# BBischof/ESRecsys

Hardware: AMD Instinct MI355X
Metric: training pairs/sec (higher is better)
Workload: dtype f32; 1 GPU; inbatch: V=1000000 x D=128 fp32 tables, B=8192, sparse Adagrad; score_precision=auto -> f16x2, ids=uniform, parallelism=single

## Files before the change

esrecsys_amd/csrc/esr_inbatch2h.hip:

```cpp
#include "esr_inbatch_mfma.h"
#include "esr_segment.h"
#include <atomic>
#include <type_traits>
#include <time.h>

namespace esr {

typedef _Float16 f16x8 __attribute__((ext_vector_type(8)));
typedef _Float16 f16x2 __attribute__((ext_vector_type(2)));

constexpr int kHLseOff = 2 * kPlaneBytes;
constexpr int kHBufBytes = kHLseOff + 4 * 256;
constexpr float kHOptHead = 4.0f;
constexpr float kHOverflow = 60000.0f;
constexpr int kHBufs = 3;
constexpr float kHPexp = 14.0f;
constexpr float kHBoundSafe = 14.0f;
constexpr int kHScaleWords = 8;

#define H_MFMA(a, b, c) __builtin_amdgcn_mfma_f32_32x32x16_f16((a), (b), (c), 0, 0, 0)
#define H_SB() __builtin_amdgcn_sched_barrier(0)
#define H_DMA_BARRIER()                                 \
  {                                                     \
    asm volatile("s_waitcnt vmcnt(0)" ::: "memory");    \
// ... 100 lines not shown
  const s16x8 both = {lo[0], lo[1], lo[2], lo[3], hi[0], hi[1], hi[2], hi[3]};
  ta[G][DB][PL] = __builtin_bit_cast(f16x8, both);
}
template <int G, class TA>
__device__ __forceinline__ void trh_frag_n(int f, TA& ta, const uint32_t (&tc)[4][2]) {
  switch (f) {
    case 0: trh_frag<G, 0>(ta, tc); break;
    case 1: trh_frag<G, 1>(ta, tc); break;
    case 2: trh_frag<G, 2>(ta, tc); break;
    case 3: trh_frag<G, 3>(ta, tc); break;
    case 4: trh_frag<G, 4>(ta, tc); break;
    case 5: trh_frag<G, 5>(ta, tc); break;
    case 6: trh_frag<G, 6>(ta, tc); break;
    default: trh_frag<G, 7>(ta, tc); break;
  }
}

template <int K>
__device__ __forceinline__ uint32_t dmah_off0(int64_t B, int64_t chunk, int t) {
  const int within = (t + 256 * K) & 511;
  const int row = within >> 4, seg = (within & 15) ^ swz16(row);
  return (uint32_t)((((int64_t)(K >> 1) * B + chunk * 32 + row) * k3D + seg * 8) * 2);
}
template <int K>
__device__ __forceinline__ void dmah_piece(const char* __restrict__ base, uint32_t off, char* buf, int w) {
  __builtin_amdgcn_global_load_lds((gptr_t)(base + off), (lptr_t)(buf + K * 4096 + w * 1024), 16, 0, 0);
}
#define H_DP(K, G, BUF) dmah_piece<K>(baseY, G, (BUF), w)
#define H_DMA_ADVANCE()                                                                    \
  {                                                                                        \
    const uint32_t step_ = (dpos + 1 == nc) ? (uint32_t)(8192 - nc * 8192) : 8192u;        \
    dpos = (dpos + 1 == nc) ? 0 : dpos + 1;                                                \
    g0 += step_; g1 += step_; g2 += step_; g3 += step_;                                    \
  }
#define H_DMA_CHUNK(BUF) { H_DP(0, g0, BUF); H_DP(1, g1, BUF); H_DP(2, g2, BUF); H_DP(3, g3, BUF); H_DMA_ADVANCE(); }

__global__ __launch_bounds__(256) void prep2h_kernel(RowSrc X0, RowSrc X1, float* __restrict__ amax,
                                                    float* __restrict__ diag) {
  __shared__ float red[8];
  const int t = threadIdx.x;
  const int64_t grow = (int64_t)blockIdx.x * 32 + (t >> 3);
  const int d0 = (t & 7) * 16;
  float mq = 0.f, mc = 0.f, dot = 0.f;
#pragma unroll
  for (int q = 0; q < 4; ++q) {
    const float4 f = rowsrc_load4(X0, grow, d0 + 4 * q);
    const float4 g = rowsrc_load4(X1, grow, d0 + 4 * q);
    mq = fmaxf(mq, fmaxf(fmaxf(fabsf(f.x), fabsf(f.y)), fmaxf(fabsf(f.z), fabsf(f.w))));
    mc = fmaxf(mc, fmaxf(fmaxf(fabsf(g.x), fabsf(g.y)), fmaxf(fabsf(g.z), fabsf(g.w))));
    dot = fmaf(f.x, g.x, fmaf(f.y, g.y, fmaf(f.z, g.z, fmaf(f.w, g.w, dot))));
  }
  dot += __shfl_xor(dot, 1, 64);
  dot += __shfl_xor(dot, 2, 64);
  dot += __shfl_xor(dot, 4, 64);
  if ((t & 7) == 0) diag[grow] = dot;
#pragma unroll
  for (int o = 32; o > 0; o >>= 1) {
    mq = fmaxf(mq, __shfl_xor(mq, o, 64));
    mc = fmaxf(mc, __shfl_xor(mc, o, 64));
  }
  if ((t & 63) == 0) { red[t >> 6] = mq; red[4 + (t >> 6)] = mc; }
  __syncthreads();
  if (t == 0) {
    amax[blockIdx.x] = fmaxf(fmaxf(red[0], red[1]), fmaxf(red[2], red[3]));
    amax[gridDim.x + blockIdx.x] = fmaxf(fmaxf(red[4], red[5]), fmaxf(red[6], red[7]));
  }
}

__device__ __forceinline__ int scale_exp(float amax) {
  if (!(amax > 0.f) || !(amax < INFINITY)) return 0;
  int x;
  frexpf(amax, &x);
  const int e = 14 - x;
  return e < -100 ? -100 : (e > 100 ? 100 : e);
}

__global__ __launch_bounds__(256) void split2h_kernel(RowSrc X0, RowSrc X1, int64_t B, _Float16* __restrict__ R0,
                                                     _Float16* __restrict__ R1, const float* __restrict__ amax,
                                                     float* __restrict__ nrm, float* __restrict__ sc,
                                                     unsigned long long* __restrict__ loss_acc,
                                                     int* __restrict__ flags, int nflags) {
  __shared__ float red[8];
  if (blockIdx.x == 0 && blockIdx.y == 1)
    for (int i = threadIdx.x; i < nflags; i += 256) flags[i] = 0;
  if (blockIdx.x == 0 && blockIdx.y == 0 && threadIdx.x <= kLossWords) {
    loss_acc[threadIdx.x * 16] = 0ull;
    if (threadIdx.x == 0) loss_acc[8] = 0ull;
  }
  const int t = threadIdx.x, nchunks = gridDim.x;
  float mq = 0.f, mc = 0.f;
  for (int i = t; i < nchunks; i += 256) {
    mq = fmaxf(mq, amax[i]);
    mc = fmaxf(mc, amax[nchunks + i]);
  }
#pragma unroll
  for (int o = 32; o > 0; o >>= 1) {
    mq = fmaxf(mq, __shfl_xor(mq, o, 64));
    mc = fmaxf(mc, __shfl_xor(mc, o, 64));
  }
  if ((t & 63) == 0) { red[t >> 6] = mq; red[4 + (t >> 6)] = mc; }
  __syncthreads();
  mq = fmaxf(fmaxf(red[0], red[1]), fmaxf(red[2], red[3]));
  mc = fmaxf(fmaxf(red[4], red[5]), fmaxf(red[6], red[7]));
  const int eq = scale_exp(mq), ec = scale_exp(mc);
  if (blockIdx.x == 0 && blockIdx.y == 0 && t == 0) {
    sc[0] = ldexpf(1.f, -(eq + ec));
    sc[1] = ldexpf(1.f, -ec);
    sc[2] = ldexpf(1.f, -(eq + (int)kHPexp));
    sc[3] = ldexpf(1.f, eq);
    sc[4] = ldexpf(1.f, ec);
  }
  const RowSrc X = blockIdx.y ? X1 : X0;
  _Float16* R = blockIdx.y ? R1 : R0;
  const float mul = ldexpf(1.f, blockIdx.y ? ec : eq);
  const int chunk = blockIdx.x;
  const int row = t >> 3, d0 = (t & 7) * 16;
  const int64_t grow = (int64_t)chunk * 32 + row;
  float v[16];
#pragma unroll
  for (int q = 0; q < 4; ++q) {
    const float4 f = rowsrc_load4(X, grow, d0 + 4 * q);
    v[4 * q] = f.x; v[4 * q + 1] = f.y; v[4 * q + 2] = f.z; v[4 * q + 3] = f.w;
  }
  {
    float ss = 0.f;
#pragma unroll
    for (int e = 0; e < 16; ++e) ss = fmaf(v[e], v[e], ss);
    ss += __shfl_xor(ss, 1, 64);
    ss += __shfl_xor(ss, 2, 64);
    ss += __shfl_xor(ss, 4, 64);
    ss = fmaxf(ss, __shfl_xor(ss, 8, 64));
    ss = fmaxf(ss, __shfl_xor(ss, 16, 64));
    ss = fmaxf(ss, __shfl_xor(ss, 32, 64));
    if ((t & 63) == 0) nrm[((int64_t)blockIdx.y * gridDim.x + chunk) * 4 + (t >> 6)] = ss;
  }
  f16x8 p[2][2];
#pragma unroll
  for (int e = 0; e < 16; ++e) {
    const float xs = v[e] * mul;
    const _Float16 a = (_Float16)xs;
    const _Float16 b = (_Float16)(xs - (float)a);
    p[0][e >> 3][e & 7] = a;
    p[1][e >> 3][e & 7] = b;
  }
#pragma unroll
  for (int pl = 0; pl < 2; ++pl) {
    f16x8* dst = reinterpret_cast<f16x8*>(R + ((int64_t)pl * B + grow) * k3D + d0);
    dst[0] = p[pl][0];
    dst[1] = p[pl][1];
  }
}

constexpr unsigned long long kPollTicks = 300000000ull;
__device__ __forceinline__ unsigned amax_code(float amax) {
  if (!(amax > 0.f)) return 0u;
  if (!(amax < INFINITY)) return 255u;
  int x;
  frexpf(amax, &x);
  return (unsigned)min(max(x + 127, 1), 254);
}
__device__ __forceinline__ int scale_exp_code(unsigned code) {
  if (code == 0u || code == 255u) return 0;
  const int e = 14 - ((int)code - 127);
  return e < -100 ? -100 : (e > 100 ? 100 : e);
}

__global__ __launch_bounds__(256) void prepsplit2h_kernel(RowSrc X0, RowSrc X1, int64_t B, _Float16* __restrict__ R0,
                                                         _Float16* __restrict__ R1,
                                                         unsigned long long* __restrict__ ent,
                                                         unsigned long long token, float* __restrict__ diag,
                                                         float* __restrict__ nrm, float* __restrict__ sc,
                                                         unsigned long long* __restrict__ loss_acc,
                                                         int* __restrict__ flags, int nflags,
                                                         float* __restrict__ copy0, float* __restrict__ copy1,
                                                         unsigned* __restrict__ czero, int two_level) {
  __shared__ float red[8];
  __shared__ unsigned cred[8];
  const int t = threadIdx.x, chunk = blockIdx.x, nchunks = gridDim.x;
  if (chunk == 0 && t <= kLossWords) {
    loss_acc[t * 16] = 0ull;
    if (t == 0) loss_acc[8] = 0ull;
  }
  if (chunk == 1 || nchunks == 1)
    for (int i = t; i < nflags; i += 256) flags[i] = 0;
  if (czero && chunk == 0 && t < 16) czero[t] = 0u;
  const int row = t >> 3, d0 = (t & 7) * 16;
  const int64_t grow = (int64_t)chunk * 32 + row;
  float vq[16], vc[16];
  {
    const int64_t rq = X0.idx ? (int64_t)X0.idx[grow] : grow;
    const int64_t rc = X1.idx ? (int64_t)X1.idx[grow] : grow;
    RowSrc Y0 = X0, Y1 = X1;
    Y0.idx = nullptr; Y1.idx = nullptr;
#pragma unroll
    for (int q = 0; q < 4; ++q) {
      const float4 f = rowsrc_load4(Y0, rq, d0 + 4 * q);
      const float4 g = rowsrc_load4(Y1, rc, d0 + 4 * q);
      vq[4 * q] = f.x; vq[4 * q + 1] = f.y; vq[4 * q + 2] = f.z; vq[4 * q + 3] = f.w;
      vc[4 * q] = g.x; vc[4 * q + 1] = g.y; vc[4 * q + 2] = g.z; vc[4 * q + 3] = g.w;
      if (copy0 && d0 + 4 * q < X0.ld) *reinterpret_cast<float4*>(copy0 + grow * X0.ld + d0 + 4 * q) = f;
      if (copy1 && d0 + 4 * q < X1.ld) *reinterpret_cast<float4*>(copy1 + grow * X1.ld + d0 + 4 * q) = g;
    }
  }
  float mq = 0.f, mc = 0.f, dot = 0.f, ssq = 0.f, ssc = 0.f;
#pragma unroll
  for (int e = 0; e < 16; ++e) {
    mq = fmaxf(mq, fabsf(vq[e]));
    mc = fmaxf(mc, fabsf(vc[e]));
    dot = fmaf(vq[e], vc[e], dot);
    ssq = fmaf(vq[e], vq[e], ssq);
    ssc = fmaf(vc[e], vc[e], ssc);
  }
  dot += __shfl_xor(dot, 1, 64); dot += __shfl_xor(dot, 2, 64); dot += __shfl_xor(dot, 4, 64);
  ssq += __shfl_xor(ssq, 1, 64); ssq += __shfl_xor(ssq, 2, 64); ssq += __shfl_xor(ssq, 4, 64);
  ssc += __shfl_xor(ssc, 1, 64); ssc += __shfl_xor(ssc, 2, 64); ssc += __shfl_xor(ssc, 4, 64);
  if ((t & 7) == 0) diag[grow] = dot;
#pragma unroll
  for (int o = 8; o < 64; o <<= 1) {
    ssq = fmaxf(ssq, __shfl_xor(ssq, o, 64));
    ssc = fmaxf(ssc, __shfl_xor(ssc, o, 64));
  }
  if ((t & 63) == 0) {
    nrm[((int64_t)0 * nchunks + chunk) * 4 + (t >> 6)] = ssq;
    nrm[((int64_t)1 * nchunks + chunk) * 4 + (t >> 6)] = ssc;
  }
#pragma unroll
  for (int o = 32; o > 0; o >>= 1) {
    mq = fmaxf(mq, __shfl_xor(mq, o, 64));
    mc = fmaxf(mc, __shfl_xor(mc, o, 64));
  }
  if ((t & 63) == 0) { red[t >> 6] = mq; red[4 + (t >> 6)] = mc; }
  __syncthreads();
  if (t == 0) {
    mq = fmaxf(fmaxf(red[0], red[1]), fmaxf(red[2], red[3]));
    mc = fmaxf(fmaxf(red[4], red[5]), fmaxf(red[6], red[7]));
    __hip_atomic_store(&ent[chunk], (token << 16) | (unsigned long long)(amax_code(mq) << 8 | amax_code(mc)),
                       __ATOMIC_RELAXED, __HIP_MEMORY_SCOPE_AGENT);
  }
  unsigned cq = 0u, cc = 0u;
  bool timed_out = false;
  const unsigned long long t_start = __builtin_amdgcn_s_memrealtime();
  const bool gatherer = chunk == 0 || !two_level;
  for (int i = gatherer ? t : (t == 0 ? nchunks : nchunks + 1); i < (gatherer ? nchunks : nchunks + 1); i += 256) {
    unsigned long long v;
    while (((v = __hip_atomic_load(&ent[i], __ATOMIC_RELAXED, __HIP_MEMORY_SCOPE_AGENT)) >> 16) != token) {
      if (__builtin_amdgcn_s_memrealtime() - t_start > kPollTicks) { timed_out = true; break; }
      __builtin_amdgcn_s_sleep(4);
    }
    cq = max(cq, (unsigned)(v >> 8) & 255u);
    cc = max(cc, (unsigned)v & 255u);
  }
  if (timed_out) atomicOr(reinterpret_cast<unsigned*>(loss_acc + 8), 1u);
#pragma unroll
  for (int o = 32; o > 0; o >>= 1) {
    cq = max(cq, (unsigned)__shfl_xor((int)cq, o, 64));
    cc = max(cc, (unsigned)__shfl_xor((int)cc, o, 64));
  }
  if ((t & 63) == 0) { cred[t >> 6] = cq; cred[4 + (t >> 6)] = cc; }
  __syncthreads();
  cq = max(max(cred[0], cred[1]), max(cred[2], cred[3]));
  cc = max(max(cred[4], cred[5]), max(cred[6], cred[7]));
  if (two_level && chunk == 0 && t == 0)
    __hip_atomic_store(&ent[nchunks], (token << 16) | (unsigned long long)(cq << 8 | cc), __ATOMIC_RELAXED,
                       __HIP_MEMORY_SCOPE_AGENT);
  const int eq = scale_exp_code(cq), ec = scale_exp_code(cc);
  if (chunk == 0 && t == 0) {
    sc[0] = ldexpf(1.f, -(eq + ec));
    sc[1] = ldexpf(1.f, -ec);
    sc[2] = ldexpf(1.f, -(eq + (int)kHPexp));
    sc[3] = ldexpf(1.f, eq);
    sc[4] = ldexpf(1.f, ec);
  }
#pragma unroll
  for (int m = 0; m < 2; ++m) {
    const float mul = ldexpf(1.f, m ? ec : eq);
    _Float16* R = m ? R1 : R0;
    f16x8 p[2][2];
#pragma unroll
    for (int e = 0; e < 16; ++e) {
      const float xs = (m ? vc[e] : vq[e]) * mul;
      const _Float16 a = (_Float16)xs;
      const _Float16 b = (_Float16)(xs - (float)a);
      p[0][e >> 3][e & 7] = a;
      p[1][e >> 3][e & 7] = b;
    }
#pragma unroll
    for (int pl = 0; pl < 2; ++pl) {
      f16x8* dst = reinterpret_cast<f16x8*>(R + ((int64_t)pl * B + grow) * k3D + d0);
      dst[0] = p[pl][0];
      dst[1] = p[pl][1];
    }
  }
}

constexpr int kHRmGroup = 4, kHRmRing = 4, kHRmOwned = 256;
template <bool FULL>
__device__ __forceinline__ float rowmax2h_sweep(const char* __restrict__ baseY, char* lds, int64_t B, int64_t c0, int nc,
                                                const f16x8 (&bx0)[2][8], const f16x8 (&bx1)[2][8], int t, int w, int j,
                                                int h) {
  constexpr int kG = FULL ? kHRmGroup / 2 : kHRmGroup;
  constexpr int kSlotChunk = (FULL ? 2 : 1) * kPlaneBytes, kSlot = kG * kSlotChunk;
  constexpr int kDmaPerGroup = kG * (FULL ? 4 : 2);
  const uint32_t g0 = dmah_off0<0>(B, c0, t), g1 = dmah_off0<1>(B, c0, t);
  const uint32_t g2 = dmah_off0<2>(B, c0, t), g3 = dmah_off0<3>(B, c0, t);
  const int ngroups = (nc + kG - 1) / kG;
#define H_RM_FETCH(GI)                                                                       \
  _Pragma("unroll") for (int k = 0; k < kG; ++k) {                                          \
    const int ch_ = min((GI) * kG + k, nc - 1);                                             \
    char* dst_ = lds + ((GI) % kHRmRing) * kSlot + k * kSlotChunk;                          \
    const uint32_t adv_ = (uint32_t)ch_ * 8192u;                                            \
    H_DP(0, g0 + adv_, dst_); H_DP(1, g1 + adv_, dst_);                                     \
    if (FULL) { H_DP(2, g2 + adv_, dst_); H_DP(3, g3 + adv_, dst_); }                       \
  }
#pragma unroll
  for (int gi = 0; gi < kHRmRing - 1; ++gi) { H_RM_FETCH(gi); }
  float ma = -INFINITY, mb = -INFINITY;
  for (int gi = 0; gi < ngroups; ++gi) {
    asm volatile("s_waitcnt vmcnt(%0)" ::"n"((kHRmRing - 2) * kDmaPerGroup) : "memory");
    __syncthreads();
    H_RM_FETCH(gi + kHRmRing - 1);
#pragma unroll
    for (int k = 0; k < kG; ++k) {
      if (gi * kG + k < nc) {
        const char* buf = lds + (gi % kHRmRing) * kSlot + k * kSlotChunk;
        f32x16 sa = {0.f, 0.f, 0.f, 0.f, 0.f, 0.f, 0.f, 0.f, 0.f, 0.f, 0.f, 0.f, 0.f, 0.f, 0.f, 0.f};
        f32x16 sb = sa;
#pragma unroll
        for (int s = 0; s < 8; ++s) {
          const int off = j * 256 + (((2 * s + h) ^ swz16(j)) << 4);
          const f16x8 a1 = *reinterpret_cast<const f16x8*>(buf + off);
          if (FULL) {
            const f16x8 a2 = *reinterpret_cast<const f16x8*>(buf + off + kPlaneBytes);
            sa = H_MFMA(a2, bx0[0][s], sa);
            sb = H_MFMA(a2, bx0[1][s], sb);
            sa = H_MFMA(a1, bx1[0][s], sa);
            sb = H_MFMA(a1, bx1[1][s], sb);
          }
          sa = H_MFMA(a1, bx0[0][s], sa);
          sb = H_MFMA(a1, bx0[1][s], sb);
        }
#pragma unroll
        for (int r = 0; r < 16; ++r) { ma = fmaxf(ma, sa[r]); mb = fmaxf(mb, sb[r]); }
      }
    }
  }
#undef H_RM_FETCH
  asm volatile("s_waitcnt vmcnt(0)" ::: "memory");
  const float mine = h == 0 ? ma : mb, other = h == 0 ? mb : ma;
  return fmaxf(mine, __shfl_xor(other, 32, 64));
}

__global__ __launch_bounds__(256) void rowmax2h_kernel(const _Float16* __restrict__ Xr, const _Float16* __restrict__ Yr,
                                                      int64_t B, int nsplit, float sl2, const float* __restrict__ nrm,
                                                      const float* __restrict__ sc, float* __restrict__ part_mr) {
  __shared__ __attribute__((aligned(16))) char lds[kHRmRing * kHRmGroup * kPlaneBytes];
  const int t = threadIdx.x, lane = t & 63;
  const int w = __builtin_amdgcn_readfirstlane(t >> 6);
  const int j = lane & 31, h = lane >> 5;
  const int ob = blockIdx.x / nsplit, split = blockIdx.x % nsplit;
  const int64_t wrow = (int64_t)ob * kHRmOwned + w * 64;
  const int64_t xrow = wrow + 32 * h + j;
  const bool live = wrow < B;
  float bound;
  {
    const int nslots = (int)(B / k3Chunk) * 4;
    float mq = 0.f, mc = 0.f;
    for (int i = t; i < nslots; i += 256) {
      mq = fmaxf(mq, nrm[i]);
      mc = fmaxf(mc, nrm[nslots + i]);
    }
#pragma unroll
    for (int o = 32; o > 0; o >>= 1) {
      mq = fmaxf(mq, __shfl_xor(mq, o, 64));
      mc = fmaxf(mc, __shfl_xor(mc, o, 64));
    }
    float* red = reinterpret_cast<float*>(lds);
    if (lane == 0) { red[w] = mq; red[4 + w] = mc; }
    __syncthreads();
    mq = fmaxf(fmaxf(red[0], red[1]), fmaxf(red[2], red[3]));
    mc = fmaxf(fmaxf(red[4], red[5]), fmaxf(red[6], red[7]));
    __syncthreads();
    bound = sqrtf(mq * mc) * fabsf(sl2);
    if (bound <= kHBoundSafe) {
      if (live) part_mr[(int64_t)split * B + xrow] = bound - kHPexp;
      return;
    }
  }
  const bool full = !(bound <= 1024.f);
  const float sl2s = sl2 * sc[0];
  const int nc = (int)(B / k3Chunk) / nsplit;
  const int64_t c0 = (int64_t)split * nc;
  const char* const baseY = reinterpret_cast<const char*>(Yr);
  f16x8 bx0[2][8], bx1[2][8];
#pragma unroll
  for (int u = 0; u < 2; ++u)
#pragma unroll
    for (int s = 0; s < 8; ++s) {
      const int64_t r = live ? wrow + 32 * u + j : 0;
      bx0[u][s] = *reinterpret_cast<const f16x8*>(Xr + r * k3D + 16 * s + 8 * h);
      bx1[u][s] = *reinterpret_cast<const f16x8*>(Xr + ((int64_t)B + r) * k3D + 16 * s + 8 * h);
      if (sl2 < 0.f) { bx0[u][s] = -bx0[u][s]; bx1[u][s] = -bx1[u][s]; }
    }
  const float m = full ? rowmax2h_sweep<true>(baseY, lds, B, c0, nc, bx0, bx1, t, w, j, h)
                       : rowmax2h_sweep<false>(baseY, lds, B, c0, nc, bx0, bx1, t, w, j, h);
  if (live) part_mr[(int64_t)split * B + xrow] = m * fabsf(sl2s) - kHPexp;
}

#ifndef H_S_ASM_LOADS
#define H_S_ASM_LOADS 1
#endif
template <int OFF>
__device__ __forceinline__ f16x8 lds_b128(uint32_t addr) {
  f16x8 v;
  asm volatile("ds_read_b128 %0, %1 offset:%2" : "=v"(v) : "v"(addr), "n"(OFF));
  return v;
}
#if H_S_ASM_LOADS
#define H_S_LD(P, OFFB) lds_b128<(P) * kPlaneBytes>(ap32_ + (uint32_t)(OFFB))
#define H_S_WAIT(N) { asm volatile("s_waitcnt lgkmcnt(%0)" ::"n"(N) : "memory"); }
#else
#define H_S_LD(P, OFFB) (*reinterpret_cast<const f16x8*>(ap0_ + (OFFB) + (P) * kPlaneBytes))
#define H_S_WAIT(N)
#endif
#define H_S_PHASE(NBUF, SA, VALU_ON)                                                                      \
  {                                                                                                       \
    _Pragma("unroll") for (int r_ = 0; r_ < 16; ++r_) SA[r_] = 0.f;                                       \
    const char* ap0_ = (NBUF) + j * 256;                                                                  \
    const uint32_t ap32_ = lds32 + (uint32_t)((NBUF) - lds) + (uint32_t)(j * 256);                        \
    (void)ap0_; (void)ap32_;                                                                              \
    const int sw_ = swz16(j);                                                                             \
    f16x8 a1_ = H_S_LD(0, (h ^ sw_) << 4);                                                                \
    f16x8 a2_ = H_S_LD(1, (h ^ sw_) << 4);                                                                \
    _Pragma("unroll") for (int s_ = 0; s_ < 8; ++s_) {                                                    \
      f16x8 n1_ = a1_, n2_ = a2_;                                                                         \
      if (s_ < 7) {                                                                                       \
        const int off_ = (((2 * (s_ + 1) + h) ^ sw_) << 4);                                               \
        n1_ = H_S_LD(0, off_);                                                                            \
        n2_ = H_S_LD(1, off_);                                                                            \
      }                                                                                                   \
      float e0_ = 0.f, e1_ = 0.f;                                                                         \
      f16x2 pa_ = {0, 0};                                                                                 \
      H_SB();                                                                                             \
      H_S_WAIT((s_ < 7 ? 2 : 0) + (((VALU_ON) && s_ >= 1) ? 2 : 0));                                      \
      H_SB();                                                                                             \
      SA = H_MFMA(a2_, bx[0][s_], SA);                                                                    \
// ... 924 lines not shown
    }
#undef CT_ROW_DMA
#undef CT_BAR
#undef CT_BAR_TOP_B
#undef CT_BAR_TOP
#undef CT_COMPUTE
#undef CT_LOAD
#undef CT_G1
#undef CT_G0
#undef CT_APPLY_FAC
#undef CT_LOAD_REFS
#undef CT_DMA_P
#undef CT_DMA_P_PIECE
#undef CT_DMA_Y
#undef CT_DMA_Y_PIECE
  };
  if (general) {
    sweep(std::true_type{});
  } else {
    sweep(std::false_type{});
    const float ce = cexp;
#pragma unroll
    for (int db = 0; db < 4; ++db)
#pragma unroll
      for (int r = 0; r < 16; ++r) acc[db][r] *= ce;
  }
  asm volatile("s_waitcnt vmcnt(0)" ::: "memory");
  __syncthreads();
  if (live) store_tile_via_lds<true>(lds + w * kTileLdsBytes, acc, part_O + ((int64_t)split * B + wrow) * k3D, lane);
}

__global__ __launch_bounds__(256) void fac2h_kernel(int64_t B, int nsplit, const float* __restrict__ part_m,
                                                   const float* __restrict__ part_l, float invl_scale,
                                                   float* __restrict__ fac, float* __restrict__ lse2 = nullptr,
                                                   float* __restrict__ lse_nat = nullptr) {
  const int64_t row = (int64_t)blockIdx.x * 256 + threadIdx.x;
  if (row >= B) return;
  float pm[8], pl[8];
#pragma unroll
  for (int s = 0; s < 8; ++s) {
    pm[s] = -INFINITY; pl[s] = 0.f;
    if (s < nsplit) {
      pm[s] = part_m[(int64_t)s * B + row];
      pl[s] = part_l[(int64_t)s * B + row];
    }
  }
  float M = pm[0], L = 0.f;
  float wt[8];
#pragma unroll
  for (int s = 1; s < 8; ++s) M = fmaxf(M, pm[s]);
#pragma unroll
  for (int s = 0; s < 8; ++s) {
    wt[s] = pm[s] == M ? 1.f : __builtin_amdgcn_exp2f(pm[s] - M);
    L = __fmaf_rn(pl[s], wt[s], L);
  }
  const float invL1 = __fdiv_rn(1.0f, L);
#pragma unroll
  for (int s = 0; s < 8; ++s)
    if (s < nsplit) fac[(int64_t)s * B + row] = __fmul_rn(__fmul_rn(invL1, invl_scale), wt[s]);
  if (lse2) {
    const float l2v = __fadd_rn(M, __builtin_amdgcn_logf(L));
    lse2[row] = l2v;
    if (lse_nat) lse_nat[row] = l2v * k3Ln2;
  }
}

constexpr int kCtExpShift = 11;
__global__ __launch_bounds__(256) void facscale2h_kernel(RowSrc X, int64_t B, int nsplit,
                                                        const float* __restrict__ part_m,
                                                        const float* __restrict__ part_l, float invl_scale,
                                                        const float* __restrict__ sc, float* __restrict__ fac,
                                                        float* __restrict__ lse2, float* __restrict__ lse_nat,
                                                        _Float16* __restrict__ Yt, int* __restrict__ cflags) {
  const int t = threadIdx.x, chunk = blockIdx.x;
  const int row = t >> 3, sl = t & 7, d0 = sl * 16;
  const int64_t grow = (int64_t)chunk * 32 + row;
  float v[16];
  {
    const int64_t r = X.idx ? (int64_t)X.idx[grow] : grow;
    RowSrc Y0 = X;
    Y0.idx = nullptr;
#pragma unroll
    for (int q = 0; q < 4; ++q) {
      const float4 f = rowsrc_load4(Y0, r, d0 + 4 * q);
      v[4 * q] = f.x; v[4 * q + 1] = f.y; v[4 * q + 2] = f.z; v[4 * q + 3] = f.w;
    }
  }
  const float pm_l = sl < nsplit ? part_m[(int64_t)sl * B + grow] : -INFINITY;
  const float pl_l = sl < nsplit ? part_l[(int64_t)sl * B + grow] : 0.f;
  float pm[8], pl[8];
  const int lane0 = (t & 63) & ~7;
#pragma unroll
  for (int s = 0; s < 8; ++s) {
    pm[s] = __shfl(pm_l, lane0 + s, 64);
    pl[s] = __shfl(pl_l, lane0 + s, 64);
  }
  float M = pm[0], L = 0.f;
  float wt[8];
#pragma unroll
  for (int s = 1; s < 8; ++s) M = fmaxf(M, pm[s]);
#pragma unroll
  for (int s = 0; s < 8; ++s) {
    wt[s] = pm[s] == M ? 1.f : __builtin_amdgcn_exp2f(pm[s] - M);
    L = __fmaf_rn(pl[s], wt[s], L);
  }
  const float invL1 = __fdiv_rn(1.0f, L);
  const float f1 = __fmul_rn(invL1, invl_scale);
  float wmine = 1.f;
#pragma unroll
  for (int s = 0; s < 8; ++s) wmine = s == sl ? wt[s] : wmine;
  const float fs = __fmul_rn(f1, wmine);
  if (sl < nsplit) {
    fac[(int64_t)sl * B + grow] = fs;
    if (fs != f1) cflags[sl] = 1;
  }
  if (sl == 0 && lse2) {
    const float l2v = __fadd_rn(M, __builtin_amdgcn_logf(L));
    lse2[grow] = l2v;
    if (lse_nat) lse_nat[grow] = l2v * k3Ln2;
  }
  const float mul = sc[3] * ldexpf(1.f, -kCtExpShift);
  float m = 0.f;
  f16x8 p[2][2];
#pragma unroll
  for (int e = 0; e < 16; ++e) {
    const float xs = __fmul_rn(v[e], f1) * mul;
    m = fmaxf(m, fabsf(xs));
    const _Float16 a = (_Float16)xs;
    const _Float16 b = (_Float16)(xs - (float)a);
    p[0][e >> 3][e & 7] = a;
    p[1][e >> 3][e & 7] = b;
  }
  m = fmaxf(m, __shfl_xor(m, 1, 64));
  m = fmaxf(m, __shfl_xor(m, 2, 64));
  m = fmaxf(m, __shfl_xor(m, 4, 64));
  if (sl < nsplit && (!(m < 60000.f) || (f1 != 0.f && m < kCtLive))) cflags[sl] = 1;
#pragma unroll
  for (int pl2 = 0; pl2 < 2; ++pl2) {
    f16x8* dst = reinterpret_cast<f16x8*>(Yt + ((int64_t)pl2 * B + grow) * k3D + d0);
    dst[0] = p[pl2][0];
    dst[1] = p[pl2][1];
  }
}

struct InbatchHWs {
  _Float16 *Qh, *Ch;
  float *part_O, *part_O2, *fac_side, *Qcopy, *Ccopy, *part_m, *part_mr, *part_l, *lse2, *fac, *Pmat, *nrm, *amax, *sc, *diag;
  int* flags;
  unsigned long long* loss_acc;
  unsigned long long* ent;
  _Float16* Qt;
  unsigned* czero;
  int* cflags;
};
constexpr int64_t kHMaxB = 16384;

static size_t inbatch2h_ws_layout(int64_t B, char* base, InbatchHWs* ws) {
  size_t off = 0;
  auto take = [&](size_t bytes) {
    char* p = base ? base + off : nullptr;
    off += align_up(bytes, 256);
    return p;
  };
  const size_t planes = (size_t)2 * B * k3D * 2;
  InbatchHWs w;
  w.Qh = (_Float16*)take(planes);
  w.Ch = (_Float16*)take(planes);
  w.part_O = (float*)take((size_t)8 * B * k3D * 4);
  w.part_O2 = (float*)take((size_t)8 * B * k3D * 4);
  w.fac_side = (float*)take((size_t)8 * B * 4);
  w.Qcopy = (float*)take((size_t)B * k3D * 4);
  w.Ccopy = (float*)take((size_t)B * k3D * 4);
  w.part_m = (float*)take((size_t)8 * B * 4);
  w.part_mr = (float*)take((size_t)8 * B * 4);
  w.part_l = (float*)take((size_t)8 * B * 4);
  w.lse2 = (float*)take((size_t)B * 4);
  w.fac = (float*)take((size_t)8 * B * 4);
  w.diag = (float*)take((size_t)B * 4);
  w.flags = (int*)take((size_t)8 * (B / k3Owned) * sizeof(int));
  w.Pmat = (float*)take((size_t)B * B * 4);
  w.loss_acc = (unsigned long long*)take(sizeof(unsigned long long) * 16 * (1 + kLossWords));
  w.nrm = (float*)take((size_t)2 * (B / k3Chunk) * 4 * sizeof(float));
  w.amax = (float*)take((size_t)2 * (B / k3Chunk) * sizeof(float));
  w.sc = (float*)take(kHScaleWords * sizeof(float));
  w.ent = (unsigned long long*)take((size_t)(B / k3Chunk + 1) * sizeof(unsigned long long));
  w.Qt = (_Float16*)take(planes);
  w.czero = (unsigned*)take(16 * sizeof(unsigned));
  w.cflags = reinterpret_cast<int*>(w.czero ? w.czero + 8 : nullptr);
  if (ws) *ws = w;
  return off;
}

static int inbatch2h_nsplit(int64_t B, int per_cu) {
  const int64_t owned_blocks = B / k3Owned, nchunks = B / k3Chunk;
  int best = 1;
  for (int s = 1; s <= 8; ++s)
    if (nchunks % s == 0 && owned_blocks * s <= 320 * per_cu) best = s;
  return best;
}

struct InbatchUpdate {
  void* tables[2];
  float* accums[2];
  int64_t row_offsets[3];
  int dtype;
  const int32_t* sorted_vids;
  const int32_t* perm;
  float* grad_rows;
  float lr, eps;
  bool skip_long;
};

static bool inbatch_events(hipEvent_t* fork, hipEvent_t* join) {
  constexpr int kMaxDev = 16;
  static thread_local hipEvent_t ev[kMaxDev][2] = {};
  int dev = 0;
  if (hipGetDevice(&dev) != hipSuccess || dev < 0 || dev >= kMaxDev) return false;
  for (int i = 0; i < 2; ++i)
    if (!ev[dev][i] && hipEventCreateWithFlags(&ev[dev][i], hipEventDisableTiming) != hipSuccess) return false;
  *fork = ev[dev][0];
  *join = ev[dev][1];
  return true;
}

}

using namespace esr;

extern "C" {

#ifdef H_TIMING
int esr_ib2h_debug_read(unsigned long long* host) {
  return (int)hipMemcpyFromSymbol(host, HIP_SYMBOL(esr_ib2h_dbg), sizeof(unsigned long long) * 8192);
}
#endif

size_t esr_inbatch2h_workspace_bytes(int64_t B, int D) {
  (void)D;
  if (B <= 0 || B > kHMaxB) return 256;
  return inbatch2h_ws_layout(B, nullptr, nullptr);
}

static int inbatch2h_run(const char* who, RowSrc Qs, RowSrc Cs, const int32_t* gq_rows, const int32_t* gc_rows, int64_t B,
                         int D, float scale, float regularization, float batch_size, float* loss, float* lse,
                         float* gQ, float* gC, void* workspace, size_t workspace_bytes, esr_stream_t stream,
                         hipStream_t side = nullptr, const InbatchUpdate* upd = nullptr) {
  if (!(B > 0 && B % k3Owned == 0 && B <= kHMaxB)) {
    set_error("%s: B=%lld must be a positive multiple of 128, at most %lld (larger batches: the bf16x3 entry point)",
              who, (long long)B, (long long)kHMaxB);
    return ESR_EINVAL;
  }
  if (!(D > 0 && D <= k3D && D % 4 == 0)) {
    set_error("%s: D=%d not supported (a multiple of 4, at most 128; wider rows: the f32 entry point)", who, D);
    return ESR_EINVAL;
  }
  if (!(Qs.base && Cs.base && loss && gQ && gC)) {
    set_error("%s: null pointer", who);
    return ESR_EINVAL;
  }
  if (batch_size == 0.f) {
    set_error("%s: batch_size must be non-zero", who);
    return ESR_EINVAL;
  }
  if ((((uintptr_t)Qs.base | (uintptr_t)Cs.base | (uintptr_t)gQ | (uintptr_t)gC) & 15) != 0) {
    set_error("%s: matrices must be 16-byte aligned", who);
    return ESR_EINVAL;
  }
  if (!workspace || workspace_bytes < esr_inbatch2h_workspace_bytes(B, D) || ((uintptr_t)workspace & 15)) {
    set_error("%s: workspace %zu bytes < %zu required (or misaligned)", who, workspace_bytes,
              esr_inbatch2h_workspace_bytes(B, D));
    return ESR_EWORKSPACE;
  }
  hipStream_t st = as_stream(stream);
  InbatchHWs ws;
  inbatch2h_ws_layout(B, (char*)workspace, &ws);
  const float inv_bs = 1.0f / batch_size, sl2 = scale * k3Log2e;
  const int nchunks = (int)(B / k3Chunk);
  const char* qcs = getenv("ESR_IB2H_Q_PER_CU");
  const int nsplit_q = inbatch2h_nsplit(B, qcs ? std::max(1, atoi(qcs)) : 2);
  const int pc_blocks = (int)cdiv(B, kCtOwned);
  int nsplit_c = 1;
  for (int sp = 1; sp <= 8; ++sp)
    if (nchunks % sp == 0 && pc_blocks * sp <= 320) nsplit_c = sp;
  const int grid_c = pc_blocks * nsplit_c;
  const int grid_q = (int)(B / k3Owned) * nsplit_q;
  const int mgrid = (int)std::min<int64_t>(k3MergeBlocks, cdiv(B, kBlock / 32));
  const char* refe = getenv("ESR_IB2H_REF");
  const int mode = (refe && refe[0] == 'r' && refe[1] == 'o') ? 0 : ((refe && refe[0] == 'r' && refe[1] == 'e') ? 2 : 1);
  const char* fe = getenv("ESR_IB2H_FUSED");
  const bool fused = !(fe && fe[0] == '0') && mode != 0;
  int nsplit_r = 1;
  hipEvent_t ev_fork = nullptr, ev_join = nullptr;
  const char* b16e = getenv("ESR_IB2H_BF16");
  const bool one_plane = fused && ((Qs.bf16 && Cs.bf16 && !(b16e && b16e[0] == 't')) || (b16e && b16e[0] == 'f'));
  const bool overlapped = fused && !one_plane && side != nullptr && side != st && inbatch_events(&ev_fork, &ev_join);
  const char* mue = getenv("ESR_IB2H_MERGE_UPDATE");
  const bool merge_upd = fused && !overlapped && upd != nullptr && upd->skip_long && D == k3D && Qs.ld == k3D &&
                         Cs.ld == k3D && !(mue && mue[0] == '0');
  auto merging_update = [&](int nsplit_of_c, const float* part_O_of_c) -> int {
    InbatchMergeArgs a;
    a.part_O[0] = ws.part_O; a.part_O[1] = part_O_of_c;
    a.nsplit[0] = nsplit_q; a.nsplit[1] = nsplit_of_c;
    a.oscale[0] = ws.sc + 1; a.oscale[1] = ws.sc + 2;
    a.partner[0] = ws.Ccopy; a.partner[1] = ws.Qcopy;
    a.part_m = ws.part_m; a.part_l = ws.part_l;
    a.B = B;
    a.scale = scale; a.lam = regularization; a.inv_bs = inv_bs;
    a.loss_acc = ws.loss_acc; a.loss_scale = 1.0 / (double)batch_size; a.loss_out = loss;
    a.zero_words = ws.ent; a.nzero = nchunks + 1;
    return inbatch_merge_update(upd->tables, upd->accums, upd->row_offsets, upd->dtype, upd->sorted_vids, upd->perm, a,
                                upd->lr, upd->eps, st);
  };
  if (fused) {
    static std::atomic<unsigned long long> call_seq{0};
    static const unsigned long long seed =
        (unsigned long long)(uintptr_t)&call_seq ^ (unsigned long long)time(nullptr) * 0x9E3779B97F4A7C15ull;
    unsigned long long z = seed + 0x9E3779B97F4A7C15ull * (call_seq.fetch_add(1) + 1);
    z = (z ^ (z >> 30)) * 0xBF58476D1CE4E5B9ull;
    z = (z ^ (z >> 27)) * 0x94D049BB133111EBull;
    const unsigned long long token = ((z ^ (z >> 31)) >> 16) | 1ull;
    const char* tle = getenv("ESR_IB2H_POLL");
    const int two_level = (tle && tle[0] == 'f') ? 0 : 1;
    ESR_KT("prepsplit2h_kernel", st,
           hipLaunchKernelGGL(prepsplit2h_kernel, dim3(nchunks), dim3(256), 0, st, Qs, Cs, B, ws.Qh, ws.Ch, ws.ent, token,
                              ws.diag, ws.nrm, ws.sc, ws.loss_acc, ws.flags, grid_q, (overlapped || merge_upd) ? ws.Qcopy : (float*)nullptr,
                              (overlapped || merge_upd) ? ws.Ccopy : (float*)nullptr, ws.czero, two_level));
    if (one_plane) {
      const int blocks1 = (int)cdiv(B, kH1Owned);
      int nsplit_1 = 1;
      for (int sp = 1; sp <= 8; ++sp)
        if (nchunks % sp == 0 && blocks1 * sp <= 320) nsplit_1 = sp;
      const int nsplit_q = nsplit_1, grid_q = blocks1 * nsplit_1;
      const char* dbg1h = getenv("ESR_IB1H_DBG");
      if (dbg1h && dbg1h[0] == '1') {
        hipLaunchKernelGGL((inbatch1h_kernel<true, 1>), dim3(grid_q), dim3(512), 0, st, (const _Float16*)ws.Qh,
                           (const _Float16*)ws.Ch, B, nsplit_q, sl2, (const float*)ws.sc, (const float*)ws.diag,
                           (const float*)nullptr, mode, ws.part_m, ws.part_O, ws.part_l);
      } else
      ESR_KT("inbatch1h_kernel_q", st,
             hipLaunchKernelGGL((inbatch1h_kernel<true>), dim3(grid_q), dim3(512), 0, st, (const _Float16*)ws.Qh,
                                (const _Float16*)ws.Ch, B, nsplit_q, sl2, (const float*)ws.sc, (const float*)ws.diag,
                                (const float*)nullptr, mode, ws.part_m, ws.part_O, ws.part_l));
      if (merge_upd) {
        ESR_KT("fac2h_kernel", st,
               hipLaunchKernelGGL(fac2h_kernel, dim3((unsigned)cdiv(B, 256)), dim3(256), 0, st, B, nsplit_q,
                                  (const float*)ws.part_m, (const float*)ws.part_l, ldexpf(1.f, (int)kHPexp), ws.fac,
                                  ws.lse2, lse));
      } else
      ESR_KT("inbatch3_merge_kernel_q", st,
             hipLaunchKernelGGL((inbatch3_merge_kernel<true>), dim3(mgrid), dim3(kBlock), 0, st, Qs, Cs, gq_rows, B,
                                nsplit_q, (const float*)ws.part_O, (const float*)ws.part_m, (const float*)ws.part_l, scale,
                                regularization, inv_bs, ws.lse2, lse, gQ, ws.loss_acc, 1.0 / (double)batch_size, loss,
                                (float*)nullptr, (const float*)(ws.sc + 1), ldexpf(1.f, (int)kHPexp), ws.fac));
      float* const part_O_1c = merge_upd ? ws.part_O2 : ws.part_O;
      if (dbg1h && (dbg1h[0] == '1' || dbg1h[0] == '2')) {
        hipLaunchKernelGGL((inbatch1h_kernel<false, 1>), dim3(grid_q), dim3(512), 0, st, (const _Float16*)ws.Ch,
                           (const _Float16*)ws.Qh, B, nsplit_q, sl2, (const float*)ws.sc, (const float*)nullptr,
                           (const float*)ws.lse2, mode, (float*)nullptr, part_O_1c, (float*)nullptr);
      } else
      ESR_KT("inbatch1h_kernel_c", st,
             hipLaunchKernelGGL((inbatch1h_kernel<false>), dim3(grid_q), dim3(512), 0, st, (const _Float16*)ws.Ch,
                                (const _Float16*)ws.Qh, B, nsplit_q, sl2, (const float*)ws.sc, (const float*)nullptr,
                                (const float*)ws.lse2, mode, (float*)nullptr, part_O_1c, (float*)nullptr));
      if (merge_upd) return merging_update(nsplit_q, part_O_1c);
      ESR_KT("inbatch3_merge_kernel_c", st,
             hipLaunchKernelGGL((inbatch3_merge_kernel<false>), dim3(mgrid), dim3(kBlock), 0, st, Cs, Qs, gc_rows, B,
                                nsplit_q, (const float*)ws.part_O, (const float*)ws.part_m, (const float*)ws.part_l, scale,
                                regularization, inv_bs, ws.lse2, (float*)nullptr, gC, ws.loss_acc,
                                1.0 / (double)batch_size, loss, (float*)nullptr, (const float*)(ws.sc + 2), 1.0f,
                                (float*)nullptr, ws.ent, nchunks + 1));
      if (upd) {
        const int rc = sparse_adagrad_range(upd->tables, upd->accums, upd->row_offsets, 2, upd->dtype, D, upd->sorted_vids,
                                            upd->perm, 2 * B, upd->grad_rows, upd->lr, upd->eps, upd->skip_long, st);
        if (rc != ESR_OK) return rc;
      }
      return check_launch(who);
    }
    ESR_KT("inbatch2h_q_kernel", st,
           hipLaunchKernelGGL((inbatch2h_q_kernel<2>), dim3(grid_q), dim3(256), 0, st, (const _Float16*)ws.Qh,
                              (const _Float16*)ws.Ch, B, nsplit_q, sl2, (const float*)ws.sc, (const float*)ws.part_mr, 1,
                              (const float*)ws.diag, mode, ws.flags, ws.part_m, ws.part_O, ws.part_l, ws.Pmat));
  } else {
  ESR_KT("prep2h_kernel", st, hipLaunchKernelGGL(prep2h_kernel, dim3(nchunks), dim3(256), 0, st, Qs, Cs, ws.amax, ws.diag));
  ESR_KT("split2h_kernel", st,
         hipLaunchKernelGGL(split2h_kernel, dim3(nchunks, 2), dim3(256), 0, st, Qs, Cs, B, ws.Qh, ws.Ch,
                            (const float*)ws.amax, ws.nrm, ws.sc, ws.loss_acc, ws.flags, grid_q));
  if (mode == 0) {
    const int rm_blocks = (int)cdiv(B, kHRmOwned);
    for (int sp = 1; sp <= 8; ++sp)
      if (nchunks % sp == 0 && rm_blocks * sp <= 320) nsplit_r = sp;
    ESR_KT("rowmax2h_kernel", st,
           hipLaunchKernelGGL(rowmax2h_kernel, dim3(rm_blocks * nsplit_r), dim3(256), 0, st, (const _Float16*)ws.Qh,
                              (const _Float16*)ws.Ch, B, nsplit_r, sl2, (const float*)ws.nrm, (const float*)ws.sc,
                              ws.part_mr));
  }
  {
    ESR_KT("inbatch2h_q_kernel", st,
           hipLaunchKernelGGL((inbatch2h_q_kernel<0>), dim3(grid_q), dim3(256), 0, st, (const _Float16*)ws.Qh,
                              (const _Float16*)ws.Ch, B, nsplit_q, sl2, (const float*)ws.sc, (const float*)ws.part_mr,
                              nsplit_r, (const float*)ws.diag, mode, ws.flags, ws.part_m, ws.part_O, ws.part_l, ws.Pmat));
    if (mode != 0)
      ESR_KT("inbatch2h_q_kernel_redo", st,
             hipLaunchKernelGGL((inbatch2h_q_kernel<1>), dim3(grid_q), dim3(256), 0, st, (const _Float16*)ws.Qh,
                                (const _Float16*)ws.Ch, B, nsplit_q, sl2, (const float*)ws.sc, (const float*)ws.part_mr,
                                nsplit_r, (const float*)ws.diag, mode, ws.flags, ws.part_m, ws.part_O, ws.part_l, ws.Pmat));
  }
  }
  hipStream_t st_q = overlapped ? side : st;
  float* const part_O_c = (overlapped || merge_upd) ? ws.part_O2 : ws.part_O;
  const RowSrc Qm = overlapped ? RowSrc{ws.Qcopy, nullptr, 0, Qs.ld} : Qs;
  const RowSrc Cm = overlapped ? RowSrc{ws.Ccopy, nullptr, 0, Cs.ld} : Cs;
  const int nc_q = nchunks / nsplit_q;
  const char* pcm = getenv("ESR_IB2H_PC");
  const int force_general = (!fused || (pcm && pcm[0] == 'g')) ? 1 : 0;
  if (overlapped) {
    if (hipEventRecord(ev_fork, st) != hipSuccess || hipStreamWaitEvent(side, ev_fork, 0) != hipSuccess) {
      set_error("%s: could not fork the side stream", who);
      return ESR_ELAUNCH;
    }
  }
  if (!force_general)
    ESR_KT("facscale2h_kernel", st,
           hipLaunchKernelGGL(facscale2h_kernel, dim3(nchunks), dim3(256), 0, st,
                              (overlapped || merge_upd) ? RowSrc{ws.Qcopy, nullptr, 0, Qs.ld} : Qs, B, nsplit_q,
                              (const float*)ws.part_m, (const float*)ws.part_l, ldexpf(1.f, (int)kHPexp),
                              (const float*)ws.sc, ws.fac, merge_upd ? ws.lse2 : (float*)nullptr,
                              merge_upd ? lse : (float*)nullptr, ws.Qt, ws.cflags));
  else if (overlapped || merge_upd)
    ESR_KT("fac2h_kernel", st,
           hipLaunchKernelGGL(fac2h_kernel, dim3((unsigned)cdiv(B, 256)), dim3(256), 0, st, B, nsplit_q,
                              (const float*)ws.part_m, (const float*)ws.part_l, ldexpf(1.f, (int)kHPexp), ws.fac,
                              merge_upd ? ws.lse2 : (float*)nullptr, merge_upd ? lse : (float*)nullptr));
  if (!merge_upd)
  ESR_KT("inbatch3_merge_kernel_q", st_q,
         hipLaunchKernelGGL((inbatch3_merge_kernel<true>), dim3(mgrid), dim3(kBlock), 0, st_q, Qm, Cm, gq_rows, B, nsplit_q,
                            (const float*)ws.part_O, (const float*)ws.part_m, (const float*)ws.part_l, scale,
                            regularization, inv_bs, ws.lse2, lse, gQ, ws.loss_acc, 1.0 / (double)batch_size, loss,
                            (float*)nullptr, (const float*)(ws.sc + 1), ldexpf(1.f, (int)kHPexp),
                            overlapped ? ws.fac_side : ws.fac));
  if (overlapped) {
    if (upd) {
      const int rc = sparse_adagrad_range(upd->tables, upd->accums, upd->row_offsets, 2, upd->dtype, D, upd->sorted_vids,
                                          upd->perm, B, upd->grad_rows, upd->lr, upd->eps, upd->skip_long, side);
      if (rc != ESR_OK) return rc;
    }
    if (hipEventRecord(ev_join, side) != hipSuccess) {
      set_error("%s: could not record the join event", who);
      return ESR_ELAUNCH;
    }
  }
  ESR_KT("inbatch2h_pct_kernel", st,
         hipLaunchKernelGGL(inbatch2h_pct_kernel, dim3(grid_c), dim3(512), 0, st, (const _Float16*)ws.Qt,
                            (const _Float16*)ws.Qh, B, nsplit_c, (const float*)ws.fac, nc_q, (const char*)ws.Pmat,
                            ldexpf(1.f, kCtExpShift), (const int*)ws.cflags, force_general, part_O_c));
  if (merge_upd) return merging_update(nsplit_c, part_O_c);
  ESR_KT("inbatch3_merge_kernel_c", st,
         hipLaunchKernelGGL((inbatch3_merge_kernel<false>), dim3(mgrid), dim3(kBlock), 0, st, Cm, Qm, gc_rows, B, nsplit_c,
                            (const float*)part_O_c, (const float*)ws.part_m, (const float*)ws.part_l, scale,
                            regularization, inv_bs, ws.lse2, (float*)nullptr, gC, ws.loss_acc,
                            1.0 / (double)batch_size, loss, (float*)nullptr, (const float*)(ws.sc + 2), 1.0f,
                            (float*)nullptr, fused ? ws.ent : (unsigned long long*)nullptr, nchunks + 1));
  if (upd) {
    const int64_t off = overlapped ? B : 0;
    const int rc = sparse_adagrad_range(upd->tables, upd->accums, upd->row_offsets, 2, upd->dtype, D,
                                        upd->sorted_vids + off, upd->perm + off, 2 * B - off, upd->grad_rows, upd->lr,
                                        upd->eps, upd->skip_long, st);
    if (rc != ESR_OK) return rc;
  }
  if (overlapped && hipStreamWaitEvent(st, ev_join, 0) != hipSuccess) {
    set_error("%s: could not join the side stream", who);
    return ESR_ELAUNCH;
  }
  return check_launch(who);
}

int esr_inbatch_softmax_fwd_bwd_f16x2(const float* Q, const float* C, int64_t B, int D, float scale,
                                      float regularization, float batch_size, float* loss, float* lse, float* gQ,
                                      float* gC, void* workspace, size_t workspace_bytes, esr_stream_t stream) {
  TraceScope trace_scope_("esr_inbatch_softmax_fwd_bwd_f16x2");
// ... 113 lines not shown
```

Measured before the change: 37.59 million pairs/s.

## Speculate prep-split scales from previous step, verify and redo in follow-up kernel

Replaces the grid-wide spin-wait that collects per-chunk amax codes with a speculative guess carried over from the previous call. The prep kernel splits rows to fp16 pairs using the guessed exponents. A new resplit kernel then reduces the true codes, records hit or miss, and only recomputes the scales and split planes when the guess was wrong. This removes the inter-block polling barrier, but adds an extra kernel launch, and a miss costs a reload and re-split of every row.

```diff
diff --git a/esrecsys_amd/csrc/esr_inbatch2h.hip b/esrecsys_amd/csrc/esr_inbatch2h.hip
--- a/esrecsys_amd/csrc/esr_inbatch2h.hip
+++ b/esrecsys_amd/csrc/esr_inbatch2h.hip
@@ -276,6 +276,7 @@
 }
 
 constexpr unsigned long long kPollTicks = 300000000ull;
+constexpr int kSpecCarried = 0, kSpecUsed = 1, kSpecHits = 2, kSpecMisses = 3, kSpecWords = 4;
 __device__ __forceinline__ unsigned amax_code(float amax) {
   if (!(amax > 0.f)) return 0u;
   if (!(amax < INFINITY)) return 255u;
@@ -289,6 +290,34 @@
   return e < -100 ? -100 : (e > 100 ? 100 : e);
 }
 
+__device__ __forceinline__ void scales2h_store(float* __restrict__ sc, int eq, int ec) {
+  sc[0] = ldexpf(1.f, -(eq + ec));
+  sc[1] = ldexpf(1.f, -ec);
+  sc[2] = ldexpf(1.f, -(eq + (int)kHPexp));
+  sc[3] = ldexpf(1.f, eq);
+  sc[4] = ldexpf(1.f, ec);
+}
+__device__ __forceinline__ void split2h_store(const float (&v)[16], int e, _Float16* __restrict__ R, int64_t B,
+                                              int64_t grow, int d0) {
+  const float mul = ldexpf(1.f, e);
+  f16x8 p[2][2];
+#pragma unroll
+  for (int k = 0; k < 16; ++k) {
+    const float xs = v[k] * mul;
+    const _Float16 a = (_Float16)xs;
+    const _Float16 b = (_Float16)(xs - (float)a);
+    p[0][k >> 3][k & 7] = a;
+    p[1][k >> 3][k & 7] = b;
+  }
+#pragma unroll
+  for (int pl = 0; pl < 2; ++pl) {
+    f16x8* dst = reinterpret_cast<f16x8*>(R + ((int64_t)pl * B + grow) * k3D + d0);
+    dst[0] = p[pl][0];
+    dst[1] = p[pl][1];
+  }
+}
+
+template <bool SPEC>
 __global__ __launch_bounds__(256) void prepsplit2h_kernel(RowSrc X0, RowSrc X1, int64_t B, _Float16* __restrict__ R0,
                                                          _Float16* __restrict__ R1,
                                                          unsigned long long* __restrict__ ent,
@@ -297,10 +326,12 @@
                                                          unsigned long long* __restrict__ loss_acc,
                                                          int* __restrict__ flags, int nflags,
                                                          float* __restrict__ copy0, float* __restrict__ copy1,
-                                                         unsigned* __restrict__ czero, int two_level) {
+                                                         unsigned* __restrict__ czero, int two_level,
+                                                         unsigned long long* __restrict__ spec) {
   __shared__ float red[8];
   __shared__ unsigned cred[8];
   const int t = threadIdx.x, chunk = blockIdx.x, nchunks = gridDim.x;
+  const unsigned guess = SPEC ? (unsigned)spec[kSpecCarried] & 0xFFFFu : 0u;
   if (chunk == 0 && t <= kLossWords) {
     loss_acc[t * 16] = 0ull;
     if (t == 0) loss_acc[8] = 0ull;
@@ -361,7 +392,11 @@
     __hip_atomic_store(&ent[chunk], (token << 16) | (unsigned long long)(amax_code(mq) << 8 | amax_code(mc)),
                        __ATOMIC_RELAXED, __HIP_MEMORY_SCOPE_AGENT);
   }
-  unsigned cq = 0u, cc = 0u;
+  unsigned cq = guess >> 8, cc = guess & 255u;
+  if (SPEC) {
+    if (chunk == 0 && t == 0) spec[kSpecUsed] = (unsigned long long)guess;
+  } else {
+  cq = 0u; cc = 0u;
   bool timed_out = false;
   const unsigned long long t_start = __builtin_amdgcn_s_memrealtime();
   const bool gatherer = chunk == 0 || !two_level;
@@ -387,34 +422,67 @@
   if (two_level && chunk == 0 && t == 0)
     __hip_atomic_store(&ent[nchunks], (token << 16) | (unsigned long long)(cq << 8 | cc), __ATOMIC_RELAXED,
                        __HIP_MEMORY_SCOPE_AGENT);
+  }
+  const int eq = scale_exp_code(cq), ec = scale_exp_code(cc);
+  if (chunk == 0 && t == 0) scales2h_store(sc, eq, ec);
+  split2h_store(vq, eq, R0, B, grow, d0);
+  split2h_store(vc, ec, R1, B, grow, d0);
+}
+
+__global__ __launch_bounds__(256) void resplit2h_kernel(RowSrc X0, RowSrc X1, int64_t B, _Float16* __restrict__ R0,
+                                                       _Float16* __restrict__ R1,
+                                                       const unsigned long long* __restrict__ ent,
+                                                       unsigned long long token, float* __restrict__ sc,
+                                                       unsigned long long* __restrict__ loss_acc,
+                                                       const float* __restrict__ copy0, const float* __restrict__ copy1,
+                                                       unsigned long long* __restrict__ spec) {
+  __shared__ unsigned cred[12];
+  const int t = threadIdx.x, chunk = blockIdx.x, nchunks = gridDim.x;
+  const unsigned used = (unsigned)spec[kSpecUsed];
+  unsigned cq = 0u, cc = 0u, stale = 0u;
+  for (int i = t; i < nchunks; i += 256) {
+    const unsigned long long v = ent[i];
+    stale |= (v >> 16) != token ? 1u : 0u;
+    cq = max(cq, (unsigned)(v >> 8) & 255u);
+    cc = max(cc, (unsigned)v & 255u);
+  }
+#pragma unroll
+  for (int o = 32; o > 0; o >>= 1) {
+    cq = max(cq, (unsigned)__shfl_xor((int)cq, o, 64));
+    cc = max(cc, (unsigned)__shfl_xor((int)cc, o, 64));
+    stale |= (unsigned)__shfl_xor((int)stale, o, 64);
+  }
+  if ((t & 63) == 0) { cred[t >> 6] = cq; cred[4 + (t >> 6)] = cc; cred[8 + (t >> 6)] = stale; }
+  __syncthreads();
+  cq = max(max(cred[0], cred[1]), max(cred[2], cred[3]));
+  cc = max(max(cred[4], cred[5]), max(cred[6], cred[7]));
+  stale = cred[8] | cred[9] | cred[10] | cred[11];
+  const unsigned codes = cq << 8 | cc;
+  const bool hit = codes == used;
   const int eq = scale_exp_code(cq), ec = scale_exp_code(cc);
   if (chunk == 0 && t == 0) {
-    sc[0] = ldexpf(1.f, -(eq + ec));
-    sc[1] = ldexpf(1.f, -ec);
-    sc[2] = ldexpf(1.f, -(eq + (int)kHPexp));
-    sc[3] = ldexpf(1.f, eq);
-    sc[4] = ldexpf(1.f, ec);
-  }
-#pragma unroll
-  for (int m = 0; m < 2; ++m) {
-    const float mul = ldexpf(1.f, m ? ec : eq);
-    _Float16* R = m ? R1 : R0;
-    f16x8 p[2][2];
-#pragma unroll
-    for (int e = 0; e < 16; ++e) {
-      const float xs = (m ? vc[e] : vq[e]) * mul;
-      const _Float16 a = (_Float16)xs;
-      const _Float16 b = (_Float16)(xs - (float)a);
-      p[0][e >> 3][e & 7] = a;
-      p[1][e >> 3][e & 7] = b;
-    }
-#pragma unroll
-    for (int pl = 0; pl < 2; ++pl) {
-      f16x8* dst = reinterpret_cast<f16x8*>(R + ((int64_t)pl * B + grow) * k3D + d0);
-      dst[0] = p[pl][0];
-      dst[1] = p[pl][1];
-    }
-  }
+    spec[kSpecCarried] = (unsigned long long)codes;
+    spec[hit ? kSpecHits : kSpecMisses] += 1ull;
+    if (stale) loss_acc[8] = 1ull;
+    if (!hit) scales2h_store(sc, eq, ec);
+  }
+  if (hit) return;
+  const int row = t >> 3, d0 = (t & 7) * 16;
+  const int64_t grow = (int64_t)chunk * 32 + row;
+  float vq[16], vc[16];
+  const int64_t rq = (!copy0 && X0.idx) ? (int64_t)X0.idx[grow] : grow;
+  const int64_t rc = (!copy1 && X1.idx) ? (int64_t)X1.idx[grow] : grow;
+  const RowSrc Y0 = copy0 ? RowSrc{copy0, nullptr, 0, X0.ld} : RowSrc{X0.base, nullptr, X0.bf16, X0.ld};
+  const RowSrc Y1 = copy1 ? RowSrc{copy1, nullptr, 0, X1.ld} : RowSrc{X1.base, nullptr, X1.bf16, X1.ld};
+#pragma unroll
+  for (int q = 0; q < 4; ++q) {
+    const float4 f = rowsrc_load4(Y0, rq, d0 + 4 * q);
+    const float4 g = rowsrc_load4(Y1, rc, d0 + 4 * q);
+    vq[4 * q] = f.x; vq[4 * q + 1] = f.y; vq[4 * q + 2] = f.z; vq[4 * q + 3] = f.w;
+    vc[4 * q] = g.x; vc[4 * q + 1] = g.y; vc[4 * q + 2] = g.z; vc[4 * q + 3] = g.w;
+  }
+  split2h_store(vq, eq, R0, B, grow, d0);
+  split2h_store(vc, ec, R1, B, grow, d0);
 }
 
 constexpr int kHRmGroup = 4, kHRmRing = 4, kHRmOwned = 256;
@@ -1645,6 +1713,7 @@
   _Float16* Qt;
   unsigned* czero;
   int* cflags;
+  unsigned long long* spec;
 };
 constexpr int64_t kHMaxB = 16384;
 
@@ -1680,6 +1749,7 @@
   w.Qt = (_Float16*)take(planes);
   w.czero = (unsigned*)take(16 * sizeof(unsigned));
   w.cflags = reinterpret_cast<int*>(w.czero ? w.czero + 8 : nullptr);
+  w.spec = (unsigned long long*)take(kSpecWords * sizeof(unsigned long long));
   if (ws) *ws = w;
   return off;
 }
@@ -1812,12 +1882,26 @@
     z = (z ^ (z >> 30)) * 0xBF58476D1CE4E5B9ull;
     z = (z ^ (z >> 27)) * 0x94D049BB133111EBull;
     const unsigned long long token = ((z ^ (z >> 31)) >> 16) | 1ull;
+    const char* spe = getenv("ESR_IB2H_SPEC");
+    const bool spec = !(spe && spe[0] == '0');
     const char* tle = getenv("ESR_IB2H_POLL");
     const int two_level = (tle && tle[0] == 'f') ? 0 : 1;
+    float* const copy_q = (overlapped || merge_upd) ? ws.Qcopy : (float*)nullptr;
+    float* const copy_c = (overlapped || merge_upd) ? ws.Ccopy : (float*)nullptr;
+    if (spec) {
+      ESR_KT("prepsplit2h_kernel", st,
+             hipLaunchKernelGGL(prepsplit2h_kernel<true>, dim3(nchunks), dim3(256), 0, st, Qs, Cs, B, ws.Qh, ws.Ch, ws.ent,
+                                token, ws.diag, ws.nrm, ws.sc, ws.loss_acc, ws.flags, grid_q, copy_q, copy_c, ws.czero, 0,
+                                ws.spec));
+      ESR_KT("resplit2h_kernel", st,
+             hipLaunchKernelGGL(resplit2h_kernel, dim3(nchunks), dim3(256), 0, st, Qs, Cs, B, ws.Qh, ws.Ch,
+                                (const unsigned long long*)ws.ent, token, ws.sc, ws.loss_acc, (const float*)copy_q,
+                                (const float*)copy_c, ws.spec));
+    } else
     ESR_KT("prepsplit2h_kernel", st,
-           hipLaunchKernelGGL(prepsplit2h_kernel, dim3(nchunks), dim3(256), 0, st, Qs, Cs, B, ws.Qh, ws.Ch, ws.ent, token,
-                              ws.diag, ws.nrm, ws.sc, ws.loss_acc, ws.flags, grid_q, (overlapped || merge_upd) ? ws.Qcopy : (float*)nullptr,
-                              (overlapped || merge_upd) ? ws.Ccopy : (float*)nullptr, ws.czero, two_level));
+           hipLaunchKernelGGL(prepsplit2h_kernel<false>, dim3(nchunks), dim3(256), 0, st, Qs, Cs, B, ws.Qh, ws.Ch, ws.ent,
+                              token, ws.diag, ws.nrm, ws.sc, ws.loss_acc, ws.flags, grid_q, copy_q, copy_c, ws.czero,
+                              two_level, (unsigned long long*)nullptr));
     if (one_plane) {
       const int blocks1 = (int)cdiv(B, kH1Owned);
       int nsplit_1 = 1;
```

After: 37.98 million pairs/s (median of 5 runs). No clear change (+1.0%).
